# haoheliu/ssr_eval

Hardware: AMD Instinct MI355X
Metric: utterance-pairs/sec (LSD+SSIM, 48kHz, n_fft=2048) (higher is better)
Workload: dtype f64

## Files before the change

__graft_entry__.py:

```python
import os
import subprocess
import sys

ROOT = os.path.dirname(os.path.abspath(__file__))
if ROOT not in sys.path:
    sys.path.insert(0, ROOT)


def build() -> None:
    from ssr_eval_amd import build as b
    b.build(force=False, verbose=True)
    sys.path.insert(0, os.path.join(ROOT, "tests"))
    import emu_lib
    emu_lib.build()
    from oracle import tl_chain
    tl_chain.build()
    try:
        build_hbm_probe()
    except Exception as e:
        print("warning: tools/ubench did not build (%s); bench.py will report peak_measured: null" % e, file=sys.stderr)
    import ssr_eval_amd
    from ssr_eval_amd import _lib
    _lib.load()


def build_hbm_probe(force: bool = False) -> str:
    src = os.path.join(ROOT, "tools", "ubench", "hbm_probe.hip")
    out = os.path.join(ROOT, "tools", "_build", "libhbmprobe.so")
    from ssr_eval_amd import build as b
    if force or not os.path.exists(out) or os.path.getmtime(src) > os.path.getmtime(out):
        os.makedirs(os.path.dirname(out), exist_ok=True)
        subprocess.check_call([b.hipcc(), "--offload-arch=gfx950", "-O3", "-std=c++17", "-fPIC", "-shared", "-o", out, src])
    src2, out2 = os.path.join(ROOT, "tools", "ubench", "fp64_mix.hip"), os.path.join(ROOT, "tools", "_build", "fp64_mix")
    if force or not os.path.exists(out2) or os.path.getmtime(src2) > os.path.getmtime(out2):
        subprocess.check_call([b.hipcc(), "--offload-arch=gfx950", "-O2", "-o", out2, src2])
    return out


def smoke() -> None:
    import numpy as np
    import torch
    assert torch.cuda.is_available(), "smoke() needs an MI355X"
    from ssr_eval_amd import AudioMetrics
    from oracle import metrics as om
    rng = np.random.default_rng(20220328)
    tgt = (0.1 * rng.standard_normal(24000)).astype(np.float32)
    est = (tgt + 0.01 * rng.standard_normal(24000).astype(np.float32)).astype(np.float32)
# ... 15 lines not shown
```

ssr_eval_amd/csrc/ssr_host.h:

```cpp
#pragma once
#include <hip/hip_runtime.h>

#include <cstdio>
#include <cstdlib>
#include <cstring>
#include <string>
#include <vector>

#include "../../include/ssr_hip.h"
#include "ssr_block.h"
#include "ssr_tables.h"

int ssr_fail(int code, const std::string& msg);
#define HIP_TRY(expr)                                                                              \
  do {                                                                                             \
    hipError_t e_ = (expr);                                                                        \
    if (e_ != hipSuccess) return ssr_fail(SSR_ERR_HIP, std::string(#expr) + ": " + hipGetErrorString(e_)); \
  } while (0)

template <typename T> struct DevTables {
  T* window = nullptr;
  T* window_h = nullptr;
  cx<T>*tw = nullptr, *wchirp = nullptr, *bfilt = nullptr, *chirp = nullptr;
};

struct ssr_plan {
  int n_fft, hop, n_bins, precision, device;
  SsrEngine eng;
  DevTables<float> f32;
  DevTables<double> f64;
  SsrEngine weng;
  DevTables<float> f32w;
  DevTables<double> f64w;
  double* window64 = nullptr;
  double* wss_tab = nullptr;
  double* wss_rcp_tab = nullptr;
  int lowpass_engine = 0;
  float *tl_wre_t = nullptr, *tl_wim_t = nullptr, *tl_ire_t = nullptr, *tl_iim_t = nullptr, *tl_w2 = nullptr;
  int tl_ldw = 0;
  std::vector<double> ex_window;
  int ex_center = 1, ex_pad_reflect = 1;
  bool ex = false;
  std::vector<void*> allocs;
};

template <typename T> inline const DevTables<T>& ssr_tables_of(const ssr_plan* pl);
template <> inline const DevTables<float>& ssr_tables_of<float>(const ssr_plan* pl) { return pl->f32; }
template <> inline const DevTables<double>& ssr_tables_of<double>(const ssr_plan* pl) { return pl->f64; }
template <typename T> inline const DevTables<T>& ssr_wave_tables_of(const ssr_plan* pl);
template <> inline const DevTables<float>& ssr_wave_tables_of<float>(const ssr_plan* pl) { return pl->f32w; }
template <> inline const DevTables<double>& ssr_wave_tables_of<double>(const ssr_plan* pl) { return pl->f64w; }

int ssr_check_plan_device(const ssr_plan* pl, bool ex_ok = false);

struct SsrLdsSlot { enum { MAX_DEV = 32 }; size_t opted[MAX_DEV] = {}; };
inline int ssr_allow_lds(const void* fn, size_t lds, SsrLdsSlot* slot) {
  if (lds <= 48 * 1024) return SSR_OK;
  int dev = 0;
  HIP_TRY(hipGetDevice(&dev));
  const bool tracked = dev >= 0 && dev < SsrLdsSlot::MAX_DEV;
  if (tracked && slot->opted[dev] >= lds) return SSR_OK;
  HIP_TRY(hipFuncSetAttribute(fn, hipFuncAttributeMaxDynamicSharedMemorySize, (int)lds));
  if (tracked) slot->opted[dev] = lds;
  return SSR_OK;
}

inline int ssr_ceil_div(int64_t a, int64_t b) { return (int)((a + b - 1) / b); }
inline size_t ssr_align256(size_t x) { return (x + 255) & ~(size_t)255; }
int ssr_target_wgs();
int ssr_units_per_chunk_for(int max_units, int n_items, int target_wgs = 0);
bool ssr_stft_uses_wave_engine(const ssr_plan* pl, bool in64);
int ssr_stft_rn_wave_radix(const ssr_plan* pl);
int ssr_pair_units_per_chunk(const ssr_plan* pl, int max_units, int n_items, bool in64);
int ssr_pair_interleave(const ssr_plan* pl, bool in64);

inline int ssr_mag_pitch(int n_bins) { return (n_bins + 3) & ~3; }
inline bool ssr_multi_fast_path(const ssr_plan* pl, bool est64) {
  if (est64) return pl->precision == SSR_F64 && ssr_stft_rn_wave_radix(pl) == 3 && pl->weng.m == 1536;
  return ssr_stft_uses_wave_engine(pl, false) || ssr_stft_rn_wave_radix(pl) != 0;
}

inline int ssr_check_pair_index(const int32_t* tgt_len, int n_tgt, const int32_t* tgt_index, int n_est, int64_t len_limit,
                                const char* len_msg, const char* count_msg = "n_tgt and n_est must be >= 0") {
  if (n_tgt < 0 || n_est < 0) return ssr_fail(SSR_ERR_INVALID_ARG, count_msg);
  if ((n_tgt > 0 && !tgt_len) || (n_est > 0 && !tgt_index)) return ssr_fail(SSR_ERR_INVALID_ARG, "null argument");
  for (int t = 0; t < n_tgt; ++t)
    if (tgt_len[t] < 0 || tgt_len[t] >= len_limit) return ssr_fail(SSR_ERR_INVALID_ARG, len_msg);
  for (int e = 0; e < n_est; ++e)
    if (tgt_index[e] < 0 || tgt_index[e] >= n_tgt) return ssr_fail(SSR_ERR_INVALID_ARG, "tgt_index out of range");
  return SSR_OK;
}
inline int ssr_upload_pair_index(const int32_t* tgt_len, int n_tgt, const int32_t* tgt_index, int n_est, int32_t* len_dev,
                                 int32_t* idx_dev, hipStream_t s) {
  if (n_tgt) HIP_TRY(hipMemcpyAsync(len_dev, tgt_len, (size_t)n_tgt * sizeof(int32_t), hipMemcpyHostToDevice, s));
  HIP_TRY(hipMemcpyAsync(idx_dev, tgt_index, (size_t)n_est * sizeof(int32_t), hipMemcpyHostToDevice, s));
  return SSR_OK;
}
template <typename F> inline void ssr_dispatch_pair_dtypes(bool tgt_f64, bool est_f64, F&& f) {
  if (!tgt_f64 && !est_f64) f(float{}, float{});
  else if (!tgt_f64) f(float{}, double{});
  else if (!est_f64) f(double{}, float{});
  else f(double{}, double{});
// ... 31 lines not shown
```

ssr_eval_amd/csrc/ssr_metrics.h:

```cpp
#pragma once
#include "ssr_stft.h"

#define SSR_SSIM_NT 64
#define SSR_SSIM_MAXCPT 6
#define SSR_SSIM_WIN 7

SSR_HD constexpr int ssr_ssim_strip_out(int cpt) { return SSR_SSIM_NT * cpt; }
SSR_HD int ssr_ssim_pick_cpt(int n_bins) {
  const int outs = n_bins - (SSR_SSIM_WIN - 1);
  if (outs <= SSR_SSIM_NT * 4) {
    int c = (outs + SSR_SSIM_NT - 1) / SSR_SSIM_NT;
    return c < 1 ? 1 : c;
  }
  int best = 4, best_waste = 1 << 30;
  for (int c = 4; c <= SSR_SSIM_MAXCPT; ++c) {
    const int w = SSR_SSIM_NT * c;
    const int waste = ((outs + w - 1) / w) * w - outs;
    if (waste < best_waste) { best_waste = waste; best = c; }
  }
  return best;
}

struct SsrSsimParams {
  const float* x;
  const float* y;
  const int64_t* frame_off;
  const int32_t* n_rows;
  int F;
  int rows_per_tile, n_row_tiles, n_strips;
  double* part;
  int pitch;
  int vi_n;
  int64_t x_plane;
};
SSR_DEV int ssr_ssim_pitch(const SsrSsimParams& p) { return p.pitch ? p.pitch : p.F; }

template <int CPT> struct SsrSsimRegs {
  double cs[CPT + 1][4];
  double s;
  float px[2][4][CPT + 1];
  float ring[SSR_SSIM_WIN][CPT + 1];
  double pxy[CPT], pb[CPT];
  float den[CPT];
};

template <int CPT> SSR_DEV int ssr_ssim_slot(int c) { return (CPT % 2 == 0) ? c + c / CPT : c; }
template <int CPT> SSR_DEV int ssr_ssim_slot_of(int tid, int d) { return (CPT % 2 == 0) ? (CPT + 1) * tid + (d + d / CPT) : CPT * tid + d; }

template <int CPT, bool CONTIG = false> struct SsrSsimLds {
  static constexpr int PW = SSR_SSIM_NT * CPT + 8 + ((CPT % 2 == 0) ? (SSR_SSIM_NT * CPT + 8) / CPT + 1 : 0);
  static constexpr int NQ = CONTIG ? 1 : 4;
  static constexpr int RW = SSR_SSIM_NT * CPT + 8;
  static constexpr size_t ring_bytes() { return CONTIG ? sizeof(float) * SSR_SSIM_WIN * RW : 0; }
  static constexpr size_t bytes() { return ring_bytes() + sizeof(double) * (NQ * PW + SSR_SSIM_NT + 16 + 8); }
  float* yring; double* col; double* sc0; double* sc1; double* res;
  SSR_MEMBER explicit SsrSsimLds(char* base) {
    yring = reinterpret_cast<float*>(base);
    col = reinterpret_cast<double*>(base + ring_bytes());
    sc0 = col + NQ * PW;
    sc1 = sc0 + SSR_SSIM_NT;
    res = sc1 + 16;
  }
};

SSR_DEV void ssr_ld4(const float* p, float* o) {
#ifdef SSR_HOST_EMU
  memcpy(o, p, 16);
#else
  typedef float f4 __attribute__((ext_vector_type(4)));
  const f4 v = *reinterpret_cast<const f4*>(p);
  o[0] = v.x; o[1] = v.y; o[2] = v.z; o[3] = v.w;
#endif
}
SSR_DEV void ssr_st4(float* p, const float* v) {
#ifdef SSR_HOST_EMU
  memcpy(p, v, 16);
// ... 99 lines not shown
#pragma unroll
  for (int i = 0; i < VC; ++i) {
    const double a = (double)R.px[SET][0][i], b = (double)R.px[SET][1][i];
    const double c = (double)R.ring[SLOT][i], dd = (double)d[i];
    R.cs[i][0] = (R.cs[i][0] + a) - c;
    R.cs[i][1] = (R.cs[i][1] + b) - dd;
    R.cs[i][2] = fma(-dd, dd, fma(-c, c, fma(b, b, fma(a, a, R.cs[i][2]))));
    R.cs[i][3] = fma(-c, dd, fma(a, b, R.cs[i][3]));
    R.ring[SLOT][i] = R.px[SET][0][i];
    ssr_touch(R.ring[SLOT][i]);
  }
}

struct SsrSsimK {
  static constexpr double n = 49.0;
  static constexpr float cov = (float)(49.0 / 48.0);
  static constexpr float C1n = (float)((0.01 * 2.0) * (0.01 * 2.0) * 49.0 * 49.0), C2n = (float)((0.03 * 2.0) * (0.03 * 2.0) * 49.0 * 49.0);
};
SSR_DEV void ssr_ssim_stage1(double sx, double sy, double& pxy, double& pp) { pxy = sx * sy; pp = fma(sx, sx, sy * sy); }
SSR_DEV float ssr_ssim_stage2f(double pp, double sq) {
  const double t2 = fma(SsrSsimK::n, sq, -pp);
  const float b1 = (float)pp + SsrSsimK::C1n;
  const float b2 = fmaf(SsrSsimK::cov, (float)t2, SsrSsimK::C2n);
  return b1 * b2;
}
SSR_DEV float ssr_ssim_stage3f(double pxy, double sxy, float b12) {
  const double t1 = fma(SsrSsimK::n, sxy, -pxy);
  const float a1 = fmaf(2.0f, (float)pxy, SsrSsimK::C1n);
  const float a2 = fmaf(2.0f * SsrSsimK::cov, (float)t1, SsrSsimK::C2n);
#ifndef SSR_HOST_EMU
  return (a1 * a2) * __builtin_amdgcn_rcpf(b12);
#else
  return (a1 * a2) / b12;
#endif
}
SSR_DEV double ssr_ssim_value(double sx, double sy, double sq, double sxy) {
  double pxy, pp;
  ssr_ssim_stage1(sx, sy, pxy, pp);
  return (double)ssr_ssim_stage3f(pxy, sxy, ssr_ssim_stage2f(pp, sq));
}

#ifndef SSR_HOST_EMU
#define SSR_SSIM_ST(arr, idx, val) (*(volatile __attribute__((address_space(3))) double*)(&(arr)[idx]) = (val))
#define SSR_SSIM_LD(arr, idx) (*(const volatile __attribute__((address_space(3))) double*)(&(arr)[idx]))
#else
#define SSR_SSIM_ST(arr, idx, val) ((arr)[idx] = (val))
#define SSR_SSIM_LD(arr, idx) ((arr)[idx])
#endif
template <int CPT, bool CONTIG, typename BLK>
SSR_BODY void ssr_ssim_body(const SsrSsimParams& p, BLK& blk, int tile, int item, char* lds_base) {
  constexpr int NT = SSR_SSIM_NT, PW = SsrSsimLds<CPT, CONTIG>::PW, VC = CPT + 1, W = SSR_SSIM_WIN;
  using Regs = SsrSsimRegs<CPT>;
  using Lds = SsrSsimLds<CPT, CONTIG>;
  Lds L(lds_base);
  const int row_tile = tile / p.n_strips, strip = tile % p.n_strips;
  const int item_v = item;
  const float* xbase = p.x;
  if (p.vi_n > 0) { xbase += (int64_t)(item / p.vi_n) * p.x_plane; item = item % p.vi_n; }
  const int T = p.n_rows[item];
  const int out_rows = T - (W - 1);
  const int r0 = row_tile * p.rows_per_tile;
  const int r1 = (r0 + p.rows_per_tile < out_rows) ? r0 + p.rows_per_tile : out_rows;
  const int c_in0 = strip * ssr_ssim_strip_out(CPT);
  const int ncol_in = (p.F - c_in0 < NT * CPT + (W - 1)) ? p.F - c_in0 : NT * CPT + (W - 1);
  const int ncol_out = ncol_in - (W - 1);
  double* part = p.part + (int64_t)item_v * p.n_row_tiles * p.n_strips + tile;
// ... 66 lines not shown
      ssr_ssim_row_apply_contig<CPT, SET, SLOT>(R, L.yring + (SLOT) * Lds::RW, tid);                                              \
      SSR_SCHED_BARRIER();                                                                                                   \
      ssr_ssim_row_load<CPT, true, SET>(p, R, tid, x, y, ssr_ssim_row_ahead(r0 + (s_) + 2, T), -1, c_in0, ncol_in);          \
      SSR_SCHED_BARRIER();    \
    });                                                                                                                      \
    if (HORIZ) {                                                                                                             \
      SSR_UNROLL for (int q = 0; q < 4; ++q) {                                                                               \
        SSR_WPHASE(blk, regs, {              \
                                \
          SSR_UNROLL for (int i = 0; i < (CPT < 6 ? CPT : 6); ++i) SSR_SSIM_ST(L.col, ssr_ssim_slot_of<CPT>(tid, i), R.cs[i][q]);     \
          L.col[ssr_ssim_slot<CPT>(NT * CPT + (tid < 7 ? tid : 7))] = R.cs[CPT][q];                                          \
        });                                                                                                                  \
        SSR_WPHASE(blk, regs, {                                                                                              \
          double v[CPT + W - 1];                                                                                             \
          SSR_UNROLL for (int d = 0; d < CPT + W - 1; ++d)                                                                   \
            v[d] = (d < CPT) ? R.cs[d < CPT ? d : 0][q]             \
                             : SSR_SSIM_LD(L.col, ssr_ssim_slot_of<CPT>(tid, d));                                           \
                                              \
          static_assert((CPT == 4 || CPT == 8) && W == 7, "window tree of the CONTIG variant");                             \
          double wq[CPT];                                                                                                    \
          {                                                                                                                  \
            const double p56 = v[5] + v[6], p78 = v[7] + v[8];                                                               \
            const double core = (v[3] + v[4]) + p56;                                                                         \
            const double wa = core + (v[1] + v[2]), wb = core + p78;                                                         \
            wq[0] = wa + v[0]; wq[1] = wa + v[7]; wq[2] = wb + v[2]; wq[3] = wb + v[9];                                      \
            if constexpr (CPT == 8) {                                                                                        \
              const double core2 = p78 + (v[9] + v[10]);                                                                     \
              const double wa2 = core2 + p56, wb2 = core2 + (v[11] + v[12]);                                                 \
              wq[4] = wa2 + v[4]; wq[5] = wa2 + v[11]; wq[6] = wb2 + v[6]; wq[7] = wb2 + v[13];                              \
            }                                                                                                                \
          }                                                                                                                  \
                                                       \
          const int j0 = tid * CPT;                                                                                          \
          float row_s = 0.0f;                                                                                                \
          SSR_UNROLL for (int i = 0; i < CPT; ++i) {                                                                         \
            if (q == 0) R.pxy[i] = wq[i];                                                                                    \
            if (q == 1) { const double sx = R.pxy[i]; ssr_ssim_stage1(sx, wq[i], R.pxy[i], R.pb[i]); }                       \
            if (q == 2) R.den[i] = ssr_ssim_stage2f(R.pb[i], wq[i]);                                                         \
            if (q == 3) {                                                                                                    \
              const float sv = ssr_ssim_stage3f(R.pxy[i], wq[i], R.den[i]);                                                  \
              row_s += (j0 + i < ncol_out) ? sv : 0.0f;                                                                      \
            }                                                                                                                \
          }                                                                                                                  \
          if (q == 3) R.s += (double)row_s;                                                                                  \
        });                                                                                                                  \
      }                                                                                                                      \
    }
    SSR_SSIM_STEP_C(0, 0, 0, false) SSR_SSIM_STEP_C(1, 1, 1, false) SSR_SSIM_STEP_C(2, 0, 2, false)
    SSR_SSIM_STEP_C(3, 1, 3, false) SSR_SSIM_STEP_C(4, 0, 4, false) SSR_SSIM_STEP_C(5, 1, 5, false)
    int s0 = W - 1;
#define SSR_SSIM_STEP_K(k) SSR_SSIM_STEP_C(s0 + (k), (k) % 2, ((k) + W - 1) % 7, true)
    for (; s0 + 14 <= n_steps; s0 += 14) {
      SSR_SSIM_STEP_K(0) SSR_SSIM_STEP_K(1) SSR_SSIM_STEP_K(2) SSR_SSIM_STEP_K(3) SSR_SSIM_STEP_K(4) SSR_SSIM_STEP_K(5) SSR_SSIM_STEP_K(6)
      SSR_SSIM_STEP_K(7) SSR_SSIM_STEP_K(8) SSR_SSIM_STEP_K(9) SSR_SSIM_STEP_K(10) SSR_SSIM_STEP_K(11) SSR_SSIM_STEP_K(12) SSR_SSIM_STEP_K(13)
    }
#define SSR_SSIM_STEP_T(k) if (s0 + (k) >= n_steps) break; SSR_SSIM_STEP_K(k)
    do {
      SSR_SSIM_STEP_T(0) SSR_SSIM_STEP_T(1) SSR_SSIM_STEP_T(2) SSR_SSIM_STEP_T(3) SSR_SSIM_STEP_T(4) SSR_SSIM_STEP_T(5) SSR_SSIM_STEP_T(6)
      SSR_SSIM_STEP_T(7) SSR_SSIM_STEP_T(8) SSR_SSIM_STEP_T(9) SSR_SSIM_STEP_T(10) SSR_SSIM_STEP_T(11) SSR_SSIM_STEP_T(12)
    } while (0);
#undef SSR_SSIM_STEP_T
#undef SSR_SSIM_STEP_K
#undef SSR_SSIM_STEP_C
  } else {
    for (int s0 = 0; s0 < n_steps; s0 += 2) {
      SSR_SSIM_STEP(s0, 0, 0)
      if (s0 + 1 < n_steps) { SSR_SSIM_STEP(s0 + 1, 1, 0) }
    }
  }
#undef SSR_SSIM_STEP
#define SSR_GET_S(q) R.s
  SSR_BLOCK_SUM(blk, regs, NT, 1, L.sc0, L.sc1, L.res, SSR_GET_S);
#undef SSR_GET_S
  SSR_PHASE(blk, regs, if (tid == 0) *part = L.res[0]);
}

struct SsrSpecRedParams {
// ... 100 lines not shown
```

ssr_eval_amd/csrc/tu_core.hip:

```cpp
#include "ssr_host.h"
#include "ssr_stft.h"

#define SSR_VERSION 200

static thread_local std::string g_err;
int ssr_fail(int code, const std::string& msg) { g_err = msg; return code; }

extern "C" const char* ssr_last_error(void) { return g_err.c_str(); }
extern "C" int ssr_version(void) { return SSR_VERSION; }

int ssr_check_plan_device(const ssr_plan* pl, bool ex_ok) {
  if (pl->ex && !ex_ok)
    return ssr_fail(SSR_ERR_UNSUPPORTED, "a plan from ssr_plan_create_ex serves ssr_stft(SSR_STFT_COMPLEX), ssr_istft and ssr_fft_lowpass only");
  int dev = -1;
  HIP_TRY(hipGetDevice(&dev));
  if (dev != pl->device)
    return ssr_fail(SSR_ERR_INVALID_ARG, "plan was created on HIP device " + std::to_string(pl->device) +
                                             " but the current device is " + std::to_string(dev));
  return SSR_OK;
}

int ssr_target_wgs() { return 4096; }

bool ssr_stft_uses_wave_engine(const ssr_plan* pl, bool in64) {
// ... 70 lines not shown
  return SSR_OK;
}

template <typename T> int ssr_launch_stft(const ssr_plan* pl, SsrStftParams<T>& p, int grid, hipStream_t s) {
  const DevTables<T>& d = ssr_tables_of<T>(pl);
  p.window = d.window_h; p.tw = d.tw; p.wchirp = d.wchirp; p.bfilt = d.bfilt; p.chirp = d.chirp;
  const bool in64 = p.a64 != nullptr;
  const bool est64_rot = in64 && (p.b64 == nullptr || p.metric_mask == 0) && sizeof(T) == 8 && ssr_stft_rn_wave_radix(pl) == 3 &&
                         pl->weng.m == 1536;
  if ((!in64 || est64_rot) && p.mode == SSR_MODE_PAIR && ssr_stft_rn_wave_radix(pl)) {
    const DevTables<T>& w = ssr_wave_tables_of<T>(pl);
    p.tw = w.tw; p.wchirp = w.wchirp; p.bfilt = w.bfilt; p.chirp = w.chirp;
    return ssr_launch_stft_rn_wave<T>(pl, p, grid, s);
  }
  if (pl->eng.radix == 3) return in64 ? ssr_launch_stft_r3_64<T>(pl, p, grid, s) : ssr_launch_stft_r3<T>(pl, p, grid, s);
  if (p.mode != SSR_MODE_PAIR) return ssr_launch_stft_single<T>(pl, p, grid, s);
  return in64 ? ssr_launch_stft_pair64<T>(pl, p, grid, s) : ssr_launch_stft_pair<T>(pl, p, grid, s);
}
template int ssr_launch_stft<float>(const ssr_plan*, SsrStftParams<float>&, int, hipStream_t);
template int ssr_launch_stft<double>(const ssr_plan*, SsrStftParams<double>&, int, hipStream_t);

extern "C" int ssr_plan_create(int n_fft, int hop, int precision, ssr_plan** out) {
  if (!out) return ssr_fail(SSR_ERR_INVALID_ARG, "plan output pointer is null");
  *out = nullptr;
  if (n_fft < 2 || hop < 1) return ssr_fail(SSR_ERR_INVALID_ARG, "n_fft must be >= 2 and hop >= 1");
  if (precision != SSR_F32 && precision != SSR_F64) return ssr_fail(SSR_ERR_INVALID_ARG, "precision must be SSR_F32 or SSR_F64");
  SsrEngine eng = ssr_pick_engine(n_fft);
  if (!eng.ok) return ssr_fail(SSR_ERR_UNSUPPORTED, "n_fft too large: Bluestein length would exceed 8192 (n_fft <= 4096)");
  ssr_plan* pl = new ssr_plan();
  pl->n_fft = n_fft; pl->hop = hop; pl->n_bins = n_fft / 2 + 1; pl->precision = precision; pl->eng = eng;
  pl->weng = ssr_pick_wave_engine(n_fft);
  int rc = SSR_OK;
  if (hipGetDevice(&pl->device) != hipSuccess) rc = ssr_fail(SSR_ERR_HIP, "hipGetDevice failed (no HIP device?)");
  if (!rc) rc = (precision == SSR_F64) ? build_dev_tables<double>(pl, pl->f64, pl->f64w) : build_dev_tables<float>(pl, pl->f32, pl->f32w);
  if (!rc) {
    SsrTables<double> t;
    ssr_build_tables<double>(n_fft, t);
    rc = upload(pl, t.window, &pl->window64);
    if (!rc && hop <= n_fft) {
      std::vector<double> tab((size_t)hop);
      for (int m = 0; m < hop; ++m) {
        double wss = 0.0;
        for (int mm = m + ((n_fft - 1 - m) / hop) * hop; mm >= m; mm -= hop) wss += t.window[mm] * t.window[mm];
        tab[m] = wss < 1e-11 ? 1e-11 : wss;
      }
      rc = upload(pl, tab, &pl->wss_tab);
      for (double& v : tab) v = 1.0 / v;
      if (!rc) rc = upload(pl, tab, &pl->wss_rcp_tab);
    }
  }
  if (rc) { ssr_plan_destroy(pl); return rc; }
  *out = pl;
  return SSR_OK;
}

extern "C" int ssr_plan_create_ex(int n_fft, int hop, const double* window, int center, int pad_mode, ssr_plan** out) {
  if (!out) return ssr_fail(SSR_ERR_INVALID_ARG, "plan output pointer is null");
  *out = nullptr;
  if (n_fft < 2 || hop < 1) return ssr_fail(SSR_ERR_INVALID_ARG, "n_fft must be >= 2 and hop >= 1");
  if (pad_mode != SSR_PAD_REFLECT && pad_mode != SSR_PAD_CONSTANT) return ssr_fail(SSR_ERR_INVALID_ARG, "pad_mode must be SSR_PAD_REFLECT or SSR_PAD_CONSTANT");
  ssr_plan* pl = new ssr_plan();
  pl->n_fft = n_fft; pl->hop = hop; pl->n_bins = n_fft / 2 + 1; pl->precision = SSR_F32;
  pl->ex = true; pl->ex_center = center ? 1 : 0; pl->ex_pad_reflect = pad_mode == SSR_PAD_REFLECT ? 1 : 0;
  if (window) pl->ex_window.assign(window, window + n_fft);
  int rc = SSR_OK;
  if (hipGetDevice(&pl->device) != hipSuccess) rc = ssr_fail(SSR_ERR_HIP, "hipGetDevice failed (no HIP device?)");
// ... 235 lines not shown
```

ssr_eval_amd/csrc/tu_metrics.hip:

```cpp
#include "ssr_host.h"
#include "ssr_metrics.h"

template <int CPT, bool CONTIG>
__global__ __launch_bounds__(SSR_SSIM_NT, 1) void k_ssim(SsrSsimParams p) {
  extern __shared__ __attribute__((aligned(16))) char smem[];
  SsrBlk blk{(int)threadIdx.x};
  const int tiles = p.n_row_tiles * p.n_strips;
  ssr_ssim_body<CPT, CONTIG>(p, blk, blockIdx.x % tiles, blockIdx.x / tiles, smem);
}


__global__ __launch_bounds__(256) void k_specred(SsrSpecRedParams p) {
  extern __shared__ __attribute__((aligned(16))) char smem[];
  SsrBlk blk{(int)threadIdx.x};
  ssr_specred_body(p, blk, blockIdx.x % p.n_chunks, blockIdx.x / p.n_chunks, smem);
}

__global__ __launch_bounds__(64) void k_finalize(SsrFinalizeParams p) {
  const int item = blockIdx.x * 64 + threadIdx.x;
  if (item < p.n_items) ssr_finalize_item(p, item);
}

struct SsimGeom { int rows_per_tile, n_row_tiles, n_strips, cpt; };
static SsimGeom ssim_geom(int max_rows, int n_bins, int n_items, bool aligned_rows) {
  SsimGeom g;
  const int out_rows = max_rows - 6 > 1 ? max_rows - 6 : 1;
  int64_t r = ((int64_t)out_rows * n_items + ssr_target_wgs() - 1) / ssr_target_wgs();
  if (r < 8) r = 8;
  if (r > 128) r = 128;
  if (r > out_rows) r = out_rows;
  g.rows_per_tile = (int)r;
  g.n_row_tiles = ssr_ceil_div(out_rows, g.rows_per_tile);
  g.cpt = ssr_ssim_pick_cpt(n_bins);
  if (aligned_rows && g.cpt != 4) {
    const int outs = n_bins - (SSR_SSIM_WIN - 1);
    if (outs > 0) {
      const int strips4 = ssr_ceil_div(outs, ssr_ssim_strip_out(4)), strips_c = ssr_ceil_div(outs, ssr_ssim_strip_out(g.cpt));
      if (strips4 * 5 * 68 < strips_c * (g.cpt + 1) * 100) g.cpt = 4;
    }
  }
  g.n_strips = n_bins > 6 ? ssr_ceil_div(n_bins - 6, ssr_ssim_strip_out(g.cpt)) : 1;
  return g;
}


struct PairWs {
  size_t off_est, off_tgt, off_part, off_ssim, total;
  int units_per_chunk, n_chunks;
  SsimGeom sg;
};
static PairWs pair_ws(const ssr_plan* pl, int n_items, int max_len, int64_t total_rows, bool in64, bool want_mag) {
  PairWs w;
  const int max_T = (int)ssr_num_frames(pl, max_len);
  w.units_per_chunk = ssr_pair_units_per_chunk(pl, max_T, n_items, in64);
  w.n_chunks = ssr_ceil_div(max_T, w.units_per_chunk);
  const int S = ssr_pair_interleave(pl, in64);
  w.n_chunks = ssr_ceil_div(w.n_chunks, S) * S;
  w.sg = ssim_geom(max_T, pl->n_bins, n_items, true);
  size_t o = 0;
  w.off_est = o; o += want_mag ? ssr_align256((size_t)total_rows * ssr_mag_pitch(pl->n_bins) * sizeof(float)) : 0;
  w.off_tgt = o; o += want_mag ? ssr_align256((size_t)total_rows * ssr_mag_pitch(pl->n_bins) * sizeof(float)) : 0;
  w.off_part = o; o += ssr_align256((size_t)n_items * w.n_chunks * SSR_NPART * sizeof(double));
  w.off_ssim = o; o += ssr_align256((size_t)n_items * w.sg.n_row_tiles * w.sg.n_strips * sizeof(double));
  w.total = o;
  return w;
}

extern "C" size_t ssr_pair_metrics_workspace_bytes_for(const ssr_plan* pl, int n_items, int max_len, int64_t total_rows,
                                                        unsigned metric_mask) {
  if (!pl || n_items <= 0) return 0;
  const bool mag = metric_mask & SSR_METRIC_SSIM;
  const size_t a = pair_ws(pl, n_items, max_len, total_rows, false, mag).total, b = pair_ws(pl, n_items, max_len, total_rows, true, mag).total;
  return (a > b ? a : b) + ssr_align256((size_t)n_items * sizeof(int32_t));
}

extern "C" size_t ssr_pair_metrics_workspace_bytes(const ssr_plan* pl, int n_items, int max_len, int64_t total_rows) {
  return ssr_pair_metrics_workspace_bytes_for(pl, n_items, max_len, total_rows, SSR_METRIC_ALL);
}

template <int CPT, bool CONTIG = false> static int launch_ssim_inst(const SsrSsimParams& p, int grid, hipStream_t s) {
  const size_t lds = SsrSsimLds<CPT, CONTIG>::bytes();
  static thread_local SsrLdsSlot slot;
  if (int rc = ssr_allow_lds((const void*)k_ssim<CPT, CONTIG>, lds, &slot)) return rc;
  hipLaunchKernelGGL((k_ssim<CPT, CONTIG>), dim3(grid), dim3(SSR_SSIM_NT), lds, s, p);
  HIP_TRY(hipGetLastError());
  return SSR_OK;
}

static int launch_ssim(const float* x, const float* y, const int64_t* frame_off, const int32_t* n_rows, int n_items,
                       int F, int pitch, const SsimGeom& g, double* part, hipStream_t s) {
  SsrSsimParams p{x, y, frame_off, n_rows, F, g.rows_per_tile, g.n_row_tiles, g.n_strips, part, pitch};
// ... 101 lines not shown
                                      const int64_t* tgt_off, const int32_t* len, const int64_t* frame_off, int n_items,
                                      int max_len, int64_t total_rows, unsigned mask, double* out, void* workspace,
                                      size_t workspace_bytes, void* stream) {
  return pair_metrics_impl(pl, nullptr, est, est_off, tgt, nullptr, tgt_off, len, frame_off, n_items, max_len, total_rows,
                           mask, out, workspace, workspace_bytes, stream, 7);
}

extern "C" int ssr_pair_metrics_f64(const ssr_plan* pl, const double* est, const int64_t* est_off, const double* tgt,
                                    const int64_t* tgt_off, const int32_t* len, const int64_t* frame_off, int n_items,
                                    int max_len, int64_t total_rows, unsigned mask, double* out, void* workspace,
                                    size_t workspace_bytes, void* stream) {
  return pair_metrics_impl(pl, nullptr, est, est_off, nullptr, tgt, tgt_off, len, frame_off, n_items, max_len, total_rows,
                           mask, out, workspace, workspace_bytes, stream, 7);
}

#include "ssr_specred_wave.h"
template <int KG> __global__ __launch_bounds__(64) void k_specred_wave(SsrSpecWaveParams p) {
  ssr_specred_wave_body<KG>(p, blockIdx.x % p.n_chunks, blockIdx.x / p.n_chunks);
}

struct MultiWs {
  PairWs w;
  size_t plane, off_est, off_tgt, off_part_a, off_part_s, off_ssim, off_rows, total;
  int spec_rows_per_chunk, spec_chunks, spec_kg, n_tiles;
  bool fast;
};
static MultiWs multi_ws(const ssr_plan* pl, int n_items, int n_keys, int max_len, int64_t total_rows, unsigned mask, bool est64 = false) {
  MultiWs m;
  const bool want_ssim = mask & SSR_METRIC_SSIM;
  m.fast = ssr_multi_fast_path(pl, est64) && n_keys > 1;
  const bool mag = want_ssim || m.fast;
  m.w = pair_ws(pl, n_items, max_len, total_rows, est64, mag);
  const int max_T = (int)ssr_num_frames(pl, max_len);
  m.w.sg = ssim_geom(max_T, pl->n_bins, m.fast ? n_items * n_keys : n_items, true);
  m.n_tiles = m.w.sg.n_row_tiles * m.w.sg.n_strips;
  m.plane = mag ? ssr_align256((size_t)total_rows * ssr_mag_pitch(pl->n_bins) * sizeof(float)) : 0;
  const int n_spec = ((n_keys - 1) / 2) * 2;
  m.spec_kg = (n_spec > 0 && n_spec % 3 == 0) ? 3 : 2;
  const int64_t groups = (int64_t)n_items * (n_spec > 0 ? n_spec / m.spec_kg : 1);
  int64_t spc = ((int64_t)16384 + groups - 1) / groups;
  if (spc > max_T / 8) spc = max_T / 8;
  if (spc < 1) spc = 1;
  m.spec_chunks = (int)spc;
  m.spec_rows_per_chunk = ssr_ceil_div(max_T, m.spec_chunks);
  m.spec_chunks = ssr_ceil_div(max_T, m.spec_rows_per_chunk);
  size_t o = 0;
  m.off_est = o; o += (size_t)n_keys * m.plane;
  m.off_tgt = o; o += m.plane;
  m.off_part_a = o; o += 2 * ssr_align256((size_t)n_items * m.w.n_chunks * SSR_NPART * sizeof(double));
  m.off_part_s = o; o += ssr_align256((size_t)n_items * n_keys * m.spec_chunks * SSR_NPART * sizeof(double));
  m.off_ssim = o; o += ssr_align256((size_t)n_items * n_keys * m.n_tiles * sizeof(double));
  m.off_rows = o; o += ssr_align256((size_t)n_items * sizeof(int32_t));
  m.total = o;
  return m;
}

extern "C" size_t ssr_pair_metrics_multi_workspace_bytes(const ssr_plan* pl, int n_items, int n_keys, int max_len, int64_t total_rows,
                                                         unsigned metric_mask) {
  if (!pl || n_items <= 0 || n_keys <= 0) return 0;
  return multi_ws(pl, n_items, n_keys, max_len, total_rows, metric_mask).total;
}

template <typename T>
static int multi_stage_stft(const ssr_plan* pl, const float* a, const double* a64, const int64_t* a_off, const float* b, const double* b64,
                            const int64_t* b_off, const int32_t* len,
                            const int64_t* frame_off, int n_items, unsigned mask, bool mag, float* out_a, float* out_b, double* part,
                            const PairWs& w, hipStream_t s) {
// ... 101 lines not shown
  if (n_spec > 0)
    HIP_TRY(finalize(red_mask ? (const double*)(ws + m.off_part_s) : nullptr, m.spec_chunks, ssim_part + (size_t)n_items * m.n_tiles, n_spec * n_items, 1));
  if (odd_last) HIP_TRY(finalize(part_last, m.w.n_chunks, ssim_part + (size_t)k * n_items * m.n_tiles, n_items, k));
  return SSR_OK;
}

extern "C" int ssr_pair_metrics_multi(const ssr_plan* pl, const float* est, const int64_t* est_off, const float* tgt, const int64_t* tgt_off,
                                      const int32_t* len, const int64_t* frame_off, int n_items, int n_keys, int max_len, int64_t total_rows,
                                      unsigned mask, double* out, void* workspace, size_t workspace_bytes, void* stream) {
  if (!est) return ssr_fail(SSR_ERR_INVALID_ARG, "null argument");
  return pair_metrics_multi_impl(pl, est, nullptr, est_off, tgt, tgt_off, len, frame_off, n_items, n_keys, max_len, total_rows, mask, out,
                                 workspace, workspace_bytes, stream);
}

extern "C" size_t ssr_pair_metrics_multi_est64_workspace_bytes(const ssr_plan* pl, int n_items, int n_keys, int max_len, int64_t total_rows,
                                                               unsigned metric_mask) {
  if (!pl || n_items <= 0 || n_keys <= 0) return 0;
  return multi_ws(pl, n_items, n_keys, max_len, total_rows, metric_mask, true).total;
}
extern "C" int ssr_pair_metrics_multi_est64(const ssr_plan* pl, const double* est, const int64_t* est_off, const float* tgt, const int64_t* tgt_off,
                                            const int32_t* len, const int64_t* frame_off, int n_items, int n_keys, int max_len,
                                            int64_t total_rows, unsigned mask, double* out, void* workspace, size_t workspace_bytes,
                                            void* stream) {
  if (!est) return ssr_fail(SSR_ERR_INVALID_ARG, "null argument");
  return pair_metrics_multi_impl(pl, nullptr, est, est_off, tgt, tgt_off, len, frame_off, n_items, n_keys, max_len, total_rows, mask, out,
                                 workspace, workspace_bytes, stream);
}

struct SpecWs { size_t off_part, off_ssim, total; int rows_per_chunk, n_chunks; SsimGeom sg; };
static SpecWs spec_ws(int n_items, int max_rows, int n_bins) {
  SpecWs w;
  w.rows_per_chunk = ssr_units_per_chunk_for(max_rows, n_items);
  w.n_chunks = ssr_ceil_div(max_rows, w.rows_per_chunk);
  w.sg = ssim_geom(max_rows, n_bins, n_items, false);
  size_t o = 0;
  w.off_part = o; o += ssr_align256((size_t)n_items * w.n_chunks * SSR_NPART * sizeof(double));
  w.off_ssim = o; o += ssr_align256((size_t)n_items * w.sg.n_row_tiles * w.sg.n_strips * sizeof(double));
  w.total = o;
  return w;
}

extern "C" size_t ssr_spectrogram_metrics_workspace_bytes(int n_items, int max_rows, int n_bins) {
  if (n_items <= 0) return 0;
  return spec_ws(n_items, max_rows, n_bins).total;
}

extern "C" int ssr_spectrogram_metrics(const float* est_sp, const float* tgt_sp, const int64_t* frame_off,
                                       const int32_t* n_rows, int n_items, int max_rows, int n_bins, unsigned mask,
                                       double* out, void* workspace, size_t workspace_bytes, void* stream) {
  if (!est_sp || !tgt_sp || !frame_off || !n_rows || !out) return ssr_fail(SSR_ERR_INVALID_ARG, "null argument");
  if (n_items <= 0) return SSR_OK;
  if ((mask & ~SSR_METRIC_ALL) || mask == 0) return ssr_fail(SSR_ERR_INVALID_ARG, "bad metric mask");
  if (max_rows < 1 || n_bins < 1) return ssr_fail(SSR_ERR_INVALID_ARG, "empty spectrogram");
  if ((int64_t)max_rows * n_bins >= ((int64_t)1 << 30))
    return ssr_fail(SSR_ERR_UNSUPPORTED, "spectrogram of 2^30 elements or more (4 GiB buffer views)");
  const bool want_ssim = mask & SSR_METRIC_SSIM;
  if (want_ssim && (max_rows < 7 || n_bins < 7)) return ssr_fail(SSR_ERR_INVALID_ARG, "win_size exceeds image extent");
  const SpecWs w = spec_ws(n_items, max_rows, n_bins);
  if (!workspace || workspace_bytes < w.total) return ssr_fail(SSR_ERR_WORKSPACE, "workspace too small");
  char* ws = (char*)workspace;
  hipStream_t s = (hipStream_t)stream;
  const bool want_red = mask & (SSR_METRIC_LSD | SSR_METRIC_SISPEC | SSR_METRIC_LOG_SISPEC);
  if (want_red) {
    SsrSpecRedParams p{est_sp, tgt_sp, frame_off, n_rows, n_bins, (int)mask, w.rows_per_chunk, w.n_chunks,
                       (double*)(ws + w.off_part)};
    hipLaunchKernelGGL(k_specred, dim3(n_items * w.n_chunks), dim3(256), SsrSpecRedLds::bytes(), s, p);
    HIP_TRY(hipGetLastError());
// ... 10 lines not shown
```

Before: 341,000.

## Pick SSIM row tiling from queried occupancy and pack SSIM stages into float2

The SSIM tile height is now chosen by a cost model that queries per-CU resident workgroups for each kernel variant at plan creation and minimises the number of waves times tile length plus a warmup term, in place of a fixed target-WG heuristic. The SSIM stage-2 and stage-3 float math is also rewritten to work on packed f2 pairs, so the den buffer becomes f2 and packed FMA/multiply can be used. The aim is fewer partial tail waves and cheaper per-column arithmetic, at the cost of an occupancy query per plan and a tiling search loop. Odd CPT values may be left unhandled by the CPT/2 loops.

New measurement: 341,500 (median of 6 runs). No clear change (+0.1%).

```diff
diff --git a/__graft_entry__.py b/__graft_entry__.py
--- a/__graft_entry__.py
+++ b/__graft_entry__.py
@@ -13,6 +13,8 @@
     sys.path.insert(0, os.path.join(ROOT, "tests"))
     import emu_lib
     emu_lib.build()
+    import ssim_geom_lib
+    ssim_geom_lib.build()
     from oracle import tl_chain
     tl_chain.build()
     try:
diff --git a/ssr_eval_amd/csrc/ssr_host.h b/ssr_eval_amd/csrc/ssr_host.h
--- a/ssr_eval_amd/csrc/ssr_host.h
+++ b/ssr_eval_amd/csrc/ssr_host.h
@@ -41,6 +41,7 @@
   std::vector<double> ex_window;
   int ex_center = 1, ex_pad_reflect = 1;
   bool ex = false;
+  int ssim_resident[7] = {};
   std::vector<void*> allocs;
 };
 
@@ -68,6 +69,7 @@
 inline int ssr_ceil_div(int64_t a, int64_t b) { return (int)((a + b - 1) / b); }
 inline size_t ssr_align256(size_t x) { return (x + 255) & ~(size_t)255; }
 int ssr_target_wgs();
+void ssr_ssim_query_residency(int device, int* resident);
 int ssr_units_per_chunk_for(int max_units, int n_items, int target_wgs = 0);
 bool ssr_stft_uses_wave_engine(const ssr_plan* pl, bool in64);
 int ssr_stft_rn_wave_radix(const ssr_plan* pl);
diff --git a/ssr_eval_amd/csrc/ssr_metrics.h b/ssr_eval_amd/csrc/ssr_metrics.h
--- a/ssr_eval_amd/csrc/ssr_metrics.h
+++ b/ssr_eval_amd/csrc/ssr_metrics.h
@@ -41,7 +41,7 @@
   float px[2][4][CPT + 1];
   float ring[SSR_SSIM_WIN][CPT + 1];
   double pxy[CPT], pb[CPT];
-  float den[CPT];
+  f2 den[(CPT + 1) / 2];
 };
 
 template <int CPT> SSR_DEV int ssr_ssim_slot(int c) { return (CPT % 2 == 0) ? c + c / CPT : c; }
@@ -207,6 +207,23 @@
   return (a1 * a2) * __builtin_amdgcn_rcpf(b12);
 #else
   return (a1 * a2) / b12;
+#endif
+}
+SSR_DEV f2 ssr_ssim_stage2f2(double pp0, double pp1, double sq0, double sq1) {
+  const double t20 = fma(SsrSsimK::n, sq0, -pp0), t21 = fma(SsrSsimK::n, sq1, -pp1);
+  const f2 b1 = f2_make((float)pp0, (float)pp1) + f2_splat(SsrSsimK::C1n);
+  const f2 b2 = f2_fma(f2_splat(SsrSsimK::cov), f2_make((float)t20, (float)t21), f2_splat(SsrSsimK::C2n));
+  return b1 * b2;
+}
+SSR_DEV f2 ssr_ssim_stage3f2(double pxy0, double pxy1, double sxy0, double sxy1, f2 b12) {
+  const double t10 = fma(SsrSsimK::n, sxy0, -pxy0), t11 = fma(SsrSsimK::n, sxy1, -pxy1);
+  const f2 a1 = f2_fma(f2_splat(2.0f), f2_make((float)pxy0, (float)pxy1), f2_splat(SsrSsimK::C1n));
+  const f2 a2 = f2_fma(f2_splat(2.0f * SsrSsimK::cov), f2_make((float)t10, (float)t11), f2_splat(SsrSsimK::C2n));
+  const f2 a12 = a1 * a2;
+#ifndef SSR_HOST_EMU
+  return a12 * f2_make(__builtin_amdgcn_rcpf(b12.x), __builtin_amdgcn_rcpf(b12.y));
+#else
+  return f2_make(a12.x / b12.x, a12.y / b12.y);
 #endif
 }
 SSR_DEV double ssr_ssim_value(double sx, double sy, double sq, double sxy) {
@@ -339,17 +356,25 @@
           }                                                                                                                  \
                                                        \
           const int j0 = tid * CPT;                                                                                          \
-          float row_s = 0.0f;                                                                                                \
           SSR_UNROLL for (int i = 0; i < CPT; ++i) {                                                                         \
             if (q == 0) R.pxy[i] = wq[i];                                                                                    \
             if (q == 1) { const double sx = R.pxy[i]; ssr_ssim_stage1(sx, wq[i], R.pxy[i], R.pb[i]); }                       \
-            if (q == 2) R.den[i] = ssr_ssim_stage2f(R.pb[i], wq[i]);                                                         \
-            if (q == 3) {                                                                                                    \
-              const float sv = ssr_ssim_stage3f(R.pxy[i], wq[i], R.den[i]);                                                  \
-              row_s += (j0 + i < ncol_out) ? sv : 0.0f;                                                                      \
+          }                                                                                                                  \
+                  \
+          if (q == 2) {                                                                                                      \
+            SSR_UNROLL for (int h = 0; h < CPT / 2; ++h)                                                                     \
+              R.den[h] = ssr_ssim_stage2f2(R.pb[2 * h], R.pb[2 * h + 1], wq[2 * h], wq[2 * h + 1]);                          \
+          }                                                                                                                  \
+          if (q == 3) {                                                                                                      \
+            float sv[CPT];                                                                                                   \
+            SSR_UNROLL for (int h = 0; h < CPT / 2; ++h) {                                                                   \
+              const f2 v2 = ssr_ssim_stage3f2(R.pxy[2 * h], R.pxy[2 * h + 1], wq[2 * h], wq[2 * h + 1], R.den[h]);           \
+              sv[2 * h] = v2.x; sv[2 * h + 1] = v2.y;                                                                        \
             }                                                                                                                \
+            float row_s = 0.0f;                                                                                              \
+            SSR_UNROLL for (int i = 0; i < CPT; ++i) row_s += (j0 + i < ncol_out) ? sv[i] : 0.0f;                            \
+            R.s += (double)row_s;                                                                                            \
           }                                                                                                                  \
-          if (q == 3) R.s += (double)row_s;                                                                                  \
         });                                                                                                                  \
       }                                                                                                                      \
     }
diff --git a/ssr_eval_amd/csrc/ssr_ssim_geom.h b/ssr_eval_amd/csrc/ssr_ssim_geom.h
--- /dev/null
+++ b/ssr_eval_amd/csrc/ssr_ssim_geom.h
@@ -0,0 +1,43 @@
+#pragma once
+#include <stdint.h>
+
+struct SsrSsimTiling { int rows_per_tile, n_row_tiles; };
+
+#define SSR_SSIM_TILE_CAP 128
+#define SSR_SSIM_TILE_FLOOR 8
+#define SSR_SSIM_WARMUP_TENTHS 18
+
+inline int ssr_ssim_out_rows(int max_rows) { return max_rows - 6 > 1 ? max_rows - 6 : 1; }
+
+inline SsrSsimTiling ssr_ssim_tiling_of(int out_rows, int rows_per_tile) {
+  return {rows_per_tile, (out_rows + rows_per_tile - 1) / rows_per_tile};
+}
+
+inline SsrSsimTiling ssr_ssim_tiling_by_target(int out_rows, int64_t n_items, int target_wgs) {
+  int64_t r = ((int64_t)out_rows * n_items + target_wgs - 1) / target_wgs;
+  if (r < SSR_SSIM_TILE_FLOOR) r = SSR_SSIM_TILE_FLOOR;
+  if (r > SSR_SSIM_TILE_CAP) r = SSR_SSIM_TILE_CAP;
+  if (r > out_rows) r = out_rows;
+  return ssr_ssim_tiling_of(out_rows, (int)r);
+}
+
+inline int64_t ssr_ssim_tiling_cost(int out_rows, int64_t n_items, int n_strips, int64_t resident, int rows_per_tile) {
+  const int64_t wgs = n_items * ((out_rows + rows_per_tile - 1) / rows_per_tile) * n_strips;
+  return ((wgs + resident - 1) / resident) * ((int64_t)rows_per_tile * 10 + SSR_SSIM_WARMUP_TENTHS);
+}
+
+inline SsrSsimTiling ssr_ssim_tiling(int out_rows, int64_t n_items, int n_strips, int resident, int target_wgs) {
+  const SsrSsimTiling base = ssr_ssim_tiling_by_target(out_rows, n_items, target_wgs);
+  if (resident <= 0 || n_items <= 0 || n_strips <= 0) return base;
+  const int lo = out_rows < SSR_SSIM_TILE_FLOOR ? out_rows : SSR_SSIM_TILE_FLOOR;
+  const int hi = out_rows < SSR_SSIM_TILE_CAP ? out_rows : SSR_SSIM_TILE_CAP;
+  int best = base.rows_per_tile;
+  int64_t best_cost = ssr_ssim_tiling_cost(out_rows, n_items, n_strips, resident, best);
+  for (int r = lo; r <= hi; ++r) {
+    const int64_t c = ssr_ssim_tiling_cost(out_rows, n_items, n_strips, resident, r);
+    const int dr = r > base.rows_per_tile ? r - base.rows_per_tile : base.rows_per_tile - r;
+    const int db = best > base.rows_per_tile ? best - base.rows_per_tile : base.rows_per_tile - best;
+    if (c < best_cost || (c == best_cost && dr < db)) { best = r; best_cost = c; }
+  }
+  return ssr_ssim_tiling_of(out_rows, best);
+}
diff --git a/ssr_eval_amd/csrc/tu_core.hip b/ssr_eval_amd/csrc/tu_core.hip
--- a/ssr_eval_amd/csrc/tu_core.hip
+++ b/ssr_eval_amd/csrc/tu_core.hip
@@ -126,6 +126,7 @@
   pl->weng = ssr_pick_wave_engine(n_fft);
   int rc = SSR_OK;
   if (hipGetDevice(&pl->device) != hipSuccess) rc = ssr_fail(SSR_ERR_HIP, "hipGetDevice failed (no HIP device?)");
+  if (!rc) ssr_ssim_query_residency(pl->device, pl->ssim_resident);
   if (!rc) rc = (precision == SSR_F64) ? build_dev_tables<double>(pl, pl->f64, pl->f64w) : build_dev_tables<float>(pl, pl->f32, pl->f32w);
   if (!rc) {
     SsrTables<double> t;
diff --git a/ssr_eval_amd/csrc/tu_metrics.hip b/ssr_eval_amd/csrc/tu_metrics.hip
--- a/ssr_eval_amd/csrc/tu_metrics.hip
+++ b/ssr_eval_amd/csrc/tu_metrics.hip
@@ -1,5 +1,6 @@
 #include "ssr_host.h"
 #include "ssr_metrics.h"
+#include "ssr_ssim_geom.h"
 
 template <int CPT, bool CONTIG>
 __global__ __launch_bounds__(SSR_SSIM_NT, 1) void k_ssim(SsrSsimParams p) {
@@ -22,15 +23,28 @@
 }
 
 struct SsimGeom { int rows_per_tile, n_row_tiles, n_strips, cpt; };
-static SsimGeom ssim_geom(int max_rows, int n_bins, int n_items, bool aligned_rows) {
+template <int CPT, bool CONTIG> static int ssim_resident_of(int n_cus) {
+  int per_cu = 0;
+  if (hipOccupancyMaxActiveBlocksPerMultiprocessor(&per_cu, k_ssim<CPT, CONTIG>, SSR_SSIM_NT, SsrSsimLds<CPT, CONTIG>::bytes()) != hipSuccess) {
+    (void)hipGetLastError();
+    return 0;
+  }
+  return per_cu > 0 ? per_cu * n_cus : 0;
+}
+void ssr_ssim_query_residency(int device, int* resident) {
+  int n_cus = 0;
+  if (hipDeviceGetAttribute(&n_cus, hipDeviceAttributeMultiprocessorCount, device) != hipSuccess || n_cus <= 0) {
+    (void)hipGetLastError();
+    return;
+  }
+  resident[0] = ssim_resident_of<4, true>(n_cus);
+  resident[1] = ssim_resident_of<1, false>(n_cus); resident[2] = ssim_resident_of<2, false>(n_cus);
+  resident[3] = ssim_resident_of<3, false>(n_cus); resident[4] = ssim_resident_of<4, false>(n_cus);
+  resident[5] = ssim_resident_of<5, false>(n_cus); resident[6] = ssim_resident_of<6, false>(n_cus);
+}
+
+static SsimGeom ssim_geom(const ssr_plan* pl, int max_rows, int n_bins, int n_items, bool aligned_rows) {
   SsimGeom g;
-  const int out_rows = max_rows - 6 > 1 ? max_rows - 6 : 1;
-  int64_t r = ((int64_t)out_rows * n_items + ssr_target_wgs() - 1) / ssr_target_wgs();
-  if (r < 8) r = 8;
-  if (r > 128) r = 128;
-  if (r > out_rows) r = out_rows;
-  g.rows_per_tile = (int)r;
-  g.n_row_tiles = ssr_ceil_div(out_rows, g.rows_per_tile);
   g.cpt = ssr_ssim_pick_cpt(n_bins);
   if (aligned_rows && g.cpt != 4) {
     const int outs = n_bins - (SSR_SSIM_WIN - 1);
@@ -40,6 +54,11 @@
     }
   }
   g.n_strips = n_bins > 6 ? ssr_ceil_div(n_bins - 6, ssr_ssim_strip_out(g.cpt)) : 1;
+  const int variant = (aligned_rows && g.cpt == 4) ? 0 : g.cpt;
+  const SsrSsimTiling t = ssr_ssim_tiling(ssr_ssim_out_rows(max_rows), n_items, g.n_strips, pl ? pl->ssim_resident[variant] : 0,
+                                          ssr_target_wgs());
+  g.rows_per_tile = t.rows_per_tile;
+  g.n_row_tiles = t.n_row_tiles;
   return g;
 }
 
@@ -56,7 +75,7 @@
   w.n_chunks = ssr_ceil_div(max_T, w.units_per_chunk);
   const int S = ssr_pair_interleave(pl, in64);
   w.n_chunks = ssr_ceil_div(w.n_chunks, S) * S;
-  w.sg = ssim_geom(max_T, pl->n_bins, n_items, true);
+  w.sg = ssim_geom(pl, max_T, pl->n_bins, n_items, true);
   size_t o = 0;
   w.off_est = o; o += want_mag ? ssr_align256((size_t)total_rows * ssr_mag_pitch(pl->n_bins) * sizeof(float)) : 0;
   w.off_tgt = o; o += want_mag ? ssr_align256((size_t)total_rows * ssr_mag_pitch(pl->n_bins) * sizeof(float)) : 0;
@@ -224,7 +243,7 @@
   const bool mag = want_ssim || m.fast;
   m.w = pair_ws(pl, n_items, max_len, total_rows, est64, mag);
   const int max_T = (int)ssr_num_frames(pl, max_len);
-  m.w.sg = ssim_geom(max_T, pl->n_bins, m.fast ? n_items * n_keys : n_items, true);
+  m.w.sg = ssim_geom(pl, max_T, pl->n_bins, m.fast ? n_items * n_keys : n_items, true);
   m.n_tiles = m.w.sg.n_row_tiles * m.w.sg.n_strips;
   m.plane = mag ? ssr_align256((size_t)total_rows * ssr_mag_pitch(pl->n_bins) * sizeof(float)) : 0;
   const int n_spec = ((n_keys - 1) / 2) * 2;
@@ -392,7 +411,7 @@
   SpecWs w;
   w.rows_per_chunk = ssr_units_per_chunk_for(max_rows, n_items);
   w.n_chunks = ssr_ceil_div(max_rows, w.rows_per_chunk);
-  w.sg = ssim_geom(max_rows, n_bins, n_items, false);
+  w.sg = ssim_geom(nullptr, max_rows, n_bins, n_items, false);
   size_t o = 0;
   w.off_part = o; o += ssr_align256((size_t)n_items * w.n_chunks * SSR_NPART * sizeof(double));
   w.off_ssim = o; o += ssr_align256((size_t)n_items * w.sg.n_row_tiles * w.sg.n_strips * sizeof(double));
```
